# lxmeng/mms_answer_selection

Hardware: AMD Instinct MI355X
Metric: QA pairs/sec (fwd+bwd) at batch 4096, 300-d; % HBM roofline (higher is better)
Workload: dtype f32

## Files before the change

mms_answer_selection_amd/csrc/euclid_math.h:

```cpp
#ifndef MMS_EUCLID_MATH_H_
#define MMS_EUCLID_MATH_H_

#include <hip/hip_runtime.h>

#include "mms_common.h"

namespace mms {

struct EuclidCoef {
  float c;
  double den;
  double rcp;
};

__device__ __forceinline__ double rcp_newton(double den) {
  double r = __builtin_amdgcn_rcp(den);
  r = __builtin_fma(__builtin_fma(-den, r, 1.0), r, r);
  r = __builtin_fma(__builtin_fma(-den, r, 1.0), r, r);
  return r;
}

__device__ __forceinline__ EuclidCoef euclid_coef(float T, float g) {
  EuclidCoef k;
  k.c = g * T * T * T;
// ... 132 lines not shown
inline void with_glove_d4(int D, F&& f) {
  switch (D) {
    case 100: f(std::integral_constant<int, 25>{}); break;
    case 200: f(std::integral_constant<int, 50>{}); break;
    case 300: f(std::integral_constant<int, 75>{}); break;
  }
}
inline bool wave_width_ok(int D) { return D <= 1024; }
inline int wave_pairs(int D) { return D <= 400 ? 2 : 1; }

template <int LPR> struct SpecPlan;
template <> struct SpecPlan<32> { static constexpr int H1 = 12, L1 = 13, H2 = 15; };
template <> struct SpecPlan<64> { static constexpr int H1 = 25, L1 = 26, H2 = 36; };

template <int LPR>
__device__ __forceinline__ float chain_sum_speculative(const float4* img4, int D4, float pred1,
                                                       float pred2, int j, int lead) {
  typedef SpecPlan<LPR> P;
  const int h4 = spec_h4(D4);
  const int seg = (j == 0) ? 0 : (j <= P::L1 ? 1 : 2);
  const int c0 = (seg == 1) ? 2 * (j - 1) - P::H1 : 2 * (j - 1 - P::L1) - P::H2;
  const int pbits = __float_as_int(seg == 1 ? pred1 : pred2);
  float2v start;
  start.x = (seg == 0) ? 0.0f : __int_as_float(pbits + c0);
  start.y = (seg == 0) ? 0.0f : __int_as_float(pbits + c0 + 1);
  __builtin_amdgcn_s_setprio(3);
  const float2v end = chain_sum_lds_pk(img4 + seg * h4, h4, start);
  const float s1 = __shfl(end.x, lead, 64);
  const int k1 = __float_as_int(s1) - __float_as_int(pred1) + P::H1;
  const bool hit1 = (k1 >= 0) && (k1 <= 2 * P::H1);
  const int l1 = lead + 1 + ((hit1 ? k1 : 0) >> 1);
  const float e1x = __shfl(end.x, l1, 64), e1y = __shfl(end.y, l1, 64);
  float s2 = (k1 & 1) ? e1y : e1x;
  if (!hit1) s2 = chain_sum_lds(img4 + h4, h4, s1);
  const int k2 = __float_as_int(s2) - __float_as_int(pred2) + P::H2;
  const bool hit2 = (k2 >= 0) && (k2 <= 2 * P::H2);
  const int l2 = lead + 1 + P::L1 + ((hit2 ? k2 : 0) >> 1);
  const float e2x = __shfl(end.x, l2, 64), e2y = __shfl(end.y, l2, 64);
  float s3 = (k2 & 1) ? e2y : e2x;
  if (!hit2) s3 = chain_sum_lds(img4 + 2 * h4, h4, s2);
  __builtin_amdgcn_s_setprio(0);
  return s3;
}

typedef __attribute__((address_space(3))) const mms_v4f lds_v4f;
__device__ __forceinline__ unsigned lds_address(const void* p) {
  return (unsigned)(size_t)(__attribute__((address_space(3))) const void*)p;
}
__device__ __forceinline__ float4 lds_read4(unsigned addr, int u) {
  const mms_v4f t = ((lds_v4f*)(size_t)addr)[u];
  return make_float4(t.x, t.y, t.z, t.w);
}

template <int H4>
struct SpecSegment {
  float4 v[H4];
  __device__ __forceinline__ void load(const float4* r4) {
#pragma unroll
    for (int u = 0; u < H4; ++u) v[u] = r4[u];
  }
  __device__ __forceinline__ float2v chain(float2v s) const {
#pragma unroll
    for (int u = 0; u < H4; ++u) {
      const float2v lo = {v[u].x, v[u].y}, hi = {v[u].z, v[u].w};
      s = s + __builtin_shufflevector(lo, lo, 0, 0);
      s = s + __builtin_shufflevector(lo, lo, 1, 1);
      s = s + __builtin_shufflevector(hi, hi, 0, 0);
      s = s + __builtin_shufflevector(hi, hi, 1, 1);
    }
    return s;
  }

  static constexpr int AHEAD = H4 < 15 ? H4 : 15;
  __device__ __forceinline__ void load_first(unsigned seg) {
#pragma unroll
    for (int u = 0; u < AHEAD; ++u) v[u] = lds_read4(seg, u);
  }
  __device__ __forceinline__ float2v chain_streamed(unsigned seg, float2v s) {
#pragma unroll
    for (int u = 0; u < H4; ++u) {
      const float2v lo = {v[u].x, v[u].y}, hi = {v[u].z, v[u].w};
      s = __builtin_shufflevector(lo, lo, 0, 0) + s;
      s = __builtin_shufflevector(lo, lo, 1, 1) + s;
      s = __builtin_shufflevector(hi, hi, 0, 0) + s;
      s = __builtin_shufflevector(hi, hi, 1, 1) + s;
      if (u + AHEAD < H4) {
        asm volatile("" : "+v"(seg) : "v"(s));
        v[u + AHEAD] = lds_read4(seg, u + AHEAD);
      }
      __builtin_amdgcn_sched_barrier(0);
    }
    return s;
  }
};

__device__ __forceinline__ int spec_seg32(int j) { return (j == 0) ? 0 : (j <= SpecPlan<32>::L1 ? 1 : 2); }

__device__ __forceinline__ float2v spec_start32(float pred1, float pred2, int j) {
  typedef SpecPlan<32> P;
  const int seg = spec_seg32(j);
  const int c0 = (seg == 1) ? 2 * (j - 1) - P::H1 : 2 * (j - 1 - P::L1) - P::H2;
  const int pbits = __float_as_int(seg == 1 ? pred1 : pred2);
  float2v start;
  start.x = (seg == 0) ? 0.0f : __int_as_float(pbits + c0);
  start.y = (seg == 0) ? 0.0f : __int_as_float(pbits + c0 + 1);
  return start;
// ... 26 lines not shown
```

mms_answer_selection_amd/csrc/simcross_rows.hip:

```cpp
#include <atomic>
#include <cstdlib>
#include <cstring>

#include "cosine_math.h"
#include "euclid_math.h"
#include "mms_internal.h"

namespace mms {

template <int NIT, int RW, bool FWD, bool BWD>
__global__ __launch_bounds__(256) void euclid_rows_wave_kernel(
    const float* __restrict__ q, const float* __restrict__ a,
    const float* __restrict__ top_in, const float* __restrict__ top_diff,
    float* __restrict__ top_out, float* __restrict__ dq, float* __restrict__ da, int N,
    int D4) {
  constexpr int LPR = 64 / RW;
  extern __shared__ float4 lds4[];
  const int wave = threadIdx.x >> 6, lane = threadIdx.x & 63;
  const int row0 = (blockIdx.x * 4 + wave) * RW;
  if (row0 >= N) return;
  const int rows = min(RW, N - row0);
  const int n4 = rows * D4;
  const size_t base4 = (size_t)row0 * D4;
  const float4* q4 = reinterpret_cast<const float4*>(q) + base4;
// ... 53 lines not shown
    wave_lds_sync();
    const float dist = chain_sum_speculative<LPR>(sq4 + grow * st4, D4, my1, my2, j, grp * LPR);
    T = 1.0f / (1.0f + sqrtf(dist));
    if (BWD) asm volatile("" : "+v"(g));
    if (j == 0 && grp < rows) top_out[row0 + grp] = T;
  }
  if (!BWD) return;

  const EuclidCoef mine = euclid_coef(T, g);
  EuclidCoef kr[RW];
#pragma unroll
  for (int r = 0; r < RW; ++r) {
    kr[r].c = __int_as_float(__builtin_amdgcn_readlane(__float_as_int(mine.c), r * LPR));
    {
      const long long dn = __double_as_longlong(mine.den), rc = __double_as_longlong(mine.rcp);
      const unsigned dlo = __builtin_amdgcn_readlane((int)(unsigned)dn, r * LPR);
      const unsigned dhi = __builtin_amdgcn_readlane((int)(unsigned)(dn >> 32), r * LPR);
      const unsigned rlo = __builtin_amdgcn_readlane((int)(unsigned)rc, r * LPR);
      const unsigned rhi = __builtin_amdgcn_readlane((int)(unsigned)(rc >> 32), r * LPR);
      kr[r].den = __longlong_as_double((long long)(((unsigned long long)dhi << 32) | dlo));
      kr[r].rcp = __longlong_as_double((long long)(((unsigned long long)rhi << 32) | rlo));
    }
  }
  float4* dq4 = reinterpret_cast<float4*>(dq) + base4;
  float4* da4 = reinterpret_cast<float4*>(da) + base4;
  float4 t[NIT];
  bool any_risky = false;
#pragma unroll
  for (int it = 0; it < NIT; ++it) {
    const int i = lane + 64 * it;
    const EuclidCoef& k = (RW == 2 && i >= D4) ? kr[RW - 1] : kr[0];
    bool risky;
    t[it] = euclid_tt4_fast(k, df[it], risky);
    any_risky |= risky && (i < n4);
  }
  if (any_risky) {
#pragma unroll
    for (int it = 0; it < NIT; ++it) {
      const int i = lane + 64 * it;
      const EuclidCoef& k = (RW == 2 && i >= D4) ? kr[RW - 1] : kr[0];
      t[it] = euclid_tt4_exact(k, df[it]);
    }
  }
#pragma unroll
  for (int it = 0; it < NIT; ++it) {
    const int i = lane + 64 * it;
    if (i >= n4) break;
    float4 o0, o1;
    o0.x = 0.f + t[it].x; o0.y = 0.f + t[it].y; o0.z = 0.f + t[it].z; o0.w = 0.f + t[it].w;
    o1.x = 0.f + (-t[it].x); o1.y = 0.f + (-t[it].y); o1.z = 0.f + (-t[it].z); o1.w = 0.f + (-t[it].w);
    stream_store(dq4 + i, o0);
    stream_store(da4 + i, o1);
  }
}

template <typename I>
__device__ __forceinline__ float4 load4(const float4* p, I i) {
  const mms_v4f v = reinterpret_cast<const mms_v4f*>(p)[i];
  return make_float4(v.x, v.y, v.z, v.w);
}

template <int D4C, int WPB, bool SHIFT, bool FULL>
__device__ __forceinline__ void euclid_pair32_forward(int N, const float* __restrict__ q, const float* __restrict__ a,
                                                      float* __restrict__ top_out, float4* lds4) {
  constexpr int NIT = (D4C + 31) / 32;
  constexpr int H4 = (D4C + 2) / 3, ST4 = 3 * H4;
  constexpr int MAXU = SHIFT ? 7 : 0;
  constexpr int P1_LAST = (H4 + MAXU - 1) / 32 < NIT - 1 ? (H4 + MAXU - 1) / 32 : NIT - 1;
  constexpr int P2_LAST = (2 * H4 + MAXU - 1) / 32 < NIT - 1 ? (2 * H4 + MAXU - 1) / 32 : NIT - 1;
  const int wave = threadIdx.x >> 6, lane = threadIdx.x & 63;
  const int grp = lane >> 5, j = lane & 31;
  const int want = (blockIdx.x * WPB + wave) * 2 + grp;
  const bool have = FULL || want < N;
  const int row = have ? want : N - 1;
  const unsigned r0 = (unsigned)row * D4C;
  const float4* q4 = reinterpret_cast<const float4*>(q) + (FULL ? 0 : (size_t)row * D4C);
  const float4* a4 = reinterpret_cast<const float4*>(a) + (FULL ? 0 : (size_t)row * D4C);
  const int u = !SHIFT ? 0
                : FULL ? (int)(((unsigned)(reinterpret_cast<size_t>(q) >> 4) + r0) & 7)
                       : (int)((reinterpret_cast<size_t>(q4) >> 4) & 7);
  const int j0 = j - u;
  const bool first_ok = !SHIFT || j0 >= 0;
  const bool last_ok = j0 + 32 * (NIT - 1) < D4C;
  auto valid_slot = [&](int it) { return (it > 0 || first_ok) && (it < NIT - 1 || last_ok); };

  float4 x[NIT], y[NIT];
#pragma unroll
  for (int it = 0; it < NIT; ++it) {
    const int i = valid_slot(it) ? j0 + 32 * it : 0;
    if constexpr (FULL) {
      const unsigned off = (r0 + (unsigned)i) * 16u;
      const char* qb = reinterpret_cast<const char*>(q4) + off;
      const char* ab = reinterpret_cast<const char*>(a4) + off;
      x[it] = load4(reinterpret_cast<const float4*>(qb), 0);
      y[it] = load4(reinterpret_cast<const float4*>(ab), 0);
    } else {
      x[it] = load4(q4, i);
      y[it] = load4(a4, i);
    }
    __builtin_amdgcn_sched_barrier(0);
  }

  float4* img = lds4 + (wave * 2 + grp) * ST4;
  unsigned seg = lds_address(img + spec_seg32(j) * H4);
  asm volatile("" : "+v"(seg));
  if (ST4 > D4C && j < ST4 - D4C) img[D4C + j] = make_float4(0.f, 0.f, 0.f, 0.f);
  float p1 = 0.f, p2 = 0.f;
  float2v start = {0.f, 0.f};
#pragma unroll
  for (int it = 0; it < NIT; ++it) {
    const bool valid = valid_slot(it);
    float4 s;
// ... 998 lines not shown
```

mms_answer_selection_amd/csrc/triplet_steps.hip:

```cpp
#include <cmath>
#include <cstdint>

#include "cosine_math.h"
#include "euclid_math.h"
#include "pairrank_math.h"
#include "mms_internal.h"

namespace mms {

constexpr int kTicketTop = 1024;
constexpr int kTicketStride = kTicketTop + 32;
constexpr int kTicketGroup = 16;
constexpr int kFxSumBits = 52;
constexpr int kFxTermBits = 10;
constexpr unsigned long long kFxPoison = 1ull << 63;
constexpr unsigned long long kFxOne = 1ull << kFxSumBits;
constexpr unsigned long long kFxSumMask = kFxOne - 1;

static thread_local int t_triplet_finish = MMS_TRIPLET_FINISH_INLAUNCH;
int triplet_finish_mode() { return t_triplet_finish; }
void set_triplet_finish_mode(int m) { t_triplet_finish = m; }

struct LossArrival {
  unsigned long long fx_sum = 0, fx_bad = 0;
  bool top_wait = false;
  unsigned long long top_old = 0, top_pay = 0;
  __device__ __forceinline__ void add(float tm, double fx_scale) {
    const bool ok = tm >= 0.f && tm < (float)(1 << kFxTermBits);
    fx_sum += ok ? (unsigned long long)((double)tm * fx_scale) : 0ull;
    fx_bad += ok ? 0ull : 1ull;
  }
  template <int WPB>
  __device__ __forceinline__ void arrive(unsigned long long* wg_arrivals, unsigned long long* __restrict__ ticket) {
    const unsigned long long pay = (1ull << 60) | (fx_bad ? kFxOne : 0ull) | fx_sum;
    const unsigned long long old = __hip_atomic_fetch_add(wg_arrivals, pay, __ATOMIC_RELAXED, __HIP_MEMORY_SCOPE_WORKGROUP);
    if ((old >> 60) == (unsigned long long)(WPB - 1)) {
      const unsigned long long wg = old + pay;
      const unsigned grp = blockIdx.x / kTicketGroup;
      const unsigned gsize = min((unsigned)kTicketGroup, gridDim.x - (unsigned)kTicketGroup * grp);
      const unsigned long long gpay = kFxOne | (wg & kFxSumMask);
      if ((wg >> kFxSumBits) & 0xffull)
        __hip_atomic_fetch_or(ticket + grp, kFxPoison, __ATOMIC_RELAXED, __HIP_MEMORY_SCOPE_AGENT);
      const unsigned long long gold = __hip_atomic_fetch_add(ticket + grp, gpay, __ATOMIC_RELAXED, __HIP_MEMORY_SCOPE_AGENT);
      if (((gold >> kFxSumBits) & 0x7ffull) == (unsigned long long)(gsize - 1)) {
        const unsigned long long g = gold + gpay;
        __hip_atomic_store(ticket + grp, 0ull, __ATOMIC_RELAXED, __HIP_MEMORY_SCOPE_AGENT);
        top_pay = kFxOne | (g & kFxSumMask);
        if (g & kFxPoison) __hip_atomic_fetch_or(ticket + kTicketTop, kFxPoison, __ATOMIC_RELAXED, __HIP_MEMORY_SCOPE_AGENT);
        top_old = __hip_atomic_fetch_add(ticket + kTicketTop, top_pay, __ATOMIC_RELAXED, __HIP_MEMORY_SCOPE_AGENT);
        top_wait = true;
      }
    }
  }
  __device__ __forceinline__ void finish(unsigned long long* __restrict__ ticket, float* __restrict__ loss, double fx_scale,
// ... 56 lines not shown
    predp1 += (i < h4) ? a4 : 0.f; predp2 += (i < 2 * h4) ? a4 : 0.f;
    predn1 += (i < h4) ? b4 : 0.f; predn2 += (i < 2 * h4) ? b4 : 0.f;
  }
  {
    const int npad = st4 - D4;
    if (lane < 2 * npad) sqp[(lane / npad) * st4 + D4 + (lane % npad)] = make_float4(0.f, 0.f, 0.f, 0.f);
  }
  const int br = lane >> 5, j = lane & 31;
  float dist;
  if (SPEC) {
    predp1 = wave_sum(predp1); predp2 = wave_sum(predp2);
    predn1 = wave_sum(predn1); predn2 = wave_sum(predn2);
    wave_lds_sync();
    dist = chain_sum_speculative<32>(br ? sqn : sqp, D4, br ? predn1 : predp1, br ? predn2 : predp2,
                                     j, br * 32);
  } else {
    wave_lds_sync();
    dist = 0.f;
    if (j == 0) {
      dist = chain_sum_lds(br ? sqn : sqp, st4, 0.f);
    }
    dist = __shfl(dist, br * 32, 64);
  }
  const float Tmine = 1.0f / (1.0f + sqrtf(dist));
  const float Tp = __shfl(Tmine, 0, 64), Tn = __shfl(Tmine, 32, 64);
  asm volatile("" : "+v"(yy));
  if (lane == 0) { s_pos[row] = Tp; s_neg[row] = Tn; }

  const PairTerm pt = pair_term(Tp, Tn, yy, margin);
  float ga, gb;
  pair_grad(yy, pt.ordered, pt.similar, s0, s1, ga, gb, hinge_ge != 0);
  if (lane == 0) partials[row] = pt.term;
  const EuclidCoef k0 = euclid_coef(Tp, ga), k1 = euclid_coef(Tn, gb);

  float4* dq4 = reinterpret_cast<float4*>(dq) + base4;
  float4* dp4 = reinterpret_cast<float4*>(dap) + base4;
  float4* dn4 = reinterpret_cast<float4*>(dan) + base4;
#pragma unroll
  for (int it = 0; it < NIT; ++it) {
    const int i = lane + 64 * it;
    if (i >= D4) break;
    const float4 tp = euclid_tt4(k0, dp[it]), tn = euclid_tt4(k1, dn[it]);
    float4 oq, op, on;
    oq.x = (0.f + tp.x) + (0.f + tn.x); oq.y = (0.f + tp.y) + (0.f + tn.y);
    oq.z = (0.f + tp.z) + (0.f + tn.z); oq.w = (0.f + tp.w) + (0.f + tn.w);
    op.x = 0.f + (-tp.x); op.y = 0.f + (-tp.y); op.z = 0.f + (-tp.z); op.w = 0.f + (-tp.w);
    on.x = 0.f + (-tn.x); on.y = 0.f + (-tn.y); on.z = 0.f + (-tn.z); on.w = 0.f + (-tn.w);
    stream_store(dq4 + i, oq);
    stream_store(dp4 + i, op);
    stream_store(dn4 + i, on);
  }
}

template <int D4C, bool EXACT, int WPB, bool INL>
__global__ __launch_bounds__(64 * WPB) void triplet32x2_kernel(
    int N, float margin, float s0, float s1, const float* __restrict__ q,
    const float* __restrict__ ap, const float* __restrict__ an, const float* __restrict__ y,
    float* __restrict__ s_pos, float* __restrict__ s_neg, float* __restrict__ partials,
    float* __restrict__ dq, float* __restrict__ dap, float* __restrict__ dan, int hinge_ge,
    unsigned long long* __restrict__ ticket, float* __restrict__ loss, double fx_scale) {
  constexpr int C = 2 * D4C;
  constexpr int NIT = (C + 63) / 64;
  constexpr int PNIT = (D4C + 31) / 32, LASTN = D4C - 32 * (PNIT - 1);
  constexpr int H4 = (D4C + 2) / 3, ST4 = 3 * H4;
  __shared__ float4 lds4[WPB * 4 * ST4];
  __shared__ unsigned long long wg_arrivals;
  const int wave = threadIdx.x >> 6, lane = threadIdx.x & 63;
  if (INL) {
    if (threadIdx.x == 0) wg_arrivals = 0;
    asm volatile("s_waitcnt lgkmcnt(0)\n\ts_barrier" ::: "memory");
  }
  const long long r0 = ((long long)blockIdx.x * WPB + wave) * 2;
  const long long total4 = (long long)N * D4C;
  const long long b4 = r0 * D4C;
  const float4* q4 = reinterpret_cast<const float4*>(q);
  const float4* p4 = reinterpret_cast<const float4*>(ap);
  const float4* m4 = reinterpret_cast<const float4*>(an);
  float yy[2];
#pragma unroll
  for (int t = 0; t < 2; ++t) yy[t] = y[min(r0 + t, (long long)N - 1)];
  float4 dp[NIT], dn[NIT];
  {
    float4 x[NIT], u[NIT], v[NIT];
#pragma unroll
    for (int it = 0; it < NIT; ++it) {
      const int i = lane + 64 * it;
      long long gi = b4 + ((NIT * 64 == C || i < C) ? i : 0);
      gi = gi < total4 ? gi : total4 - 1;
      x[it] = q4[gi]; u[it] = p4[gi]; v[it] = m4[gi];
    }
    float4* img = lds4 + (size_t)wave * 4 * ST4;
#pragma unroll
    for (int it = 0; it < NIT; ++it) {
      const int i = lane + 64 * it;
      dp[it].x = x[it].x - u[it].x; dp[it].y = x[it].y - u[it].y;
      dp[it].z = x[it].z - u[it].z; dp[it].w = x[it].w - u[it].w;
      dn[it].x = x[it].x - v[it].x; dn[it].y = x[it].y - v[it].y;
      dn[it].z = x[it].z - v[it].z; dn[it].w = x[it].w - v[it].w;
      float4 a, b;
      a.x = dp[it].x * dp[it].x; a.y = dp[it].y * dp[it].y;
      a.z = dp[it].z * dp[it].z; a.w = dp[it].w * dp[it].w;
      b.x = dn[it].x * dn[it].x; b.y = dn[it].y * dn[it].y;
      b.z = dn[it].z * dn[it].z; b.w = dn[it].w * dn[it].w;
      if (NIT * 64 == C || i < C) {
        const int t = i >= D4C ? 1 : 0, c = i - t * D4C;
        img[(2 * t) * ST4 + c] = a;
        img[(2 * t + 1) * ST4 + c] = b;
      }
    }
    if constexpr (ST4 > D4C) {
      if (lane < 4 * (ST4 - D4C))
        img[(lane / (ST4 - D4C)) * ST4 + D4C + lane % (ST4 - D4C)] = make_float4(0.f, 0.f, 0.f, 0.f);
    }
  }
  asm volatile("" : "+v"(yy[0]), "+v"(yy[1]));
  wave_lds_sync();

  const int br = lane >> 5, j = lane & 31;
  float4* dq4 = reinterpret_cast<float4*>(dq);
  float4* dp4 = reinterpret_cast<float4*>(dap);
  float4* dn4 = reinterpret_cast<float4*>(dan);
  constexpr bool LATE = INL;
  LossArrival arr;
  EuclidCoef k0[2], k1[2];
  float c0[2] = {0.f, 0.f}, c1[2] = {0.f, 0.f}, rr0[2] = {0.f, 0.f}, rr1[2] = {0.f, 0.f};
  auto store_pass = [&](int t) {
    const bool have = r0 + t < N;
#pragma unroll
    for (int it = 0; it < NIT; ++it) {
      if (64 * it >= (t + 1) * D4C || 64 * it + 63 < t * D4C) continue;
      const int i = lane + 64 * it;
      const bool mine = have && i >= t * D4C && i < (t + 1) * D4C;
      float4 tp, tn;
      if (EXACT) { tp = euclid_tt4(k0[t], dp[it]); tn = euclid_tt4(k1[t], dn[it]); }
      else {
        tp.x = (c0[t] * dp[it].x) * rr0[t]; tp.y = (c0[t] * dp[it].y) * rr0[t];
        tp.z = (c0[t] * dp[it].z) * rr0[t]; tp.w = (c0[t] * dp[it].w) * rr0[t];
        tn.x = (c1[t] * dn[it].x) * rr1[t]; tn.y = (c1[t] * dn[it].y) * rr1[t];
        tn.z = (c1[t] * dn[it].z) * rr1[t]; tn.w = (c1[t] * dn[it].w) * rr1[t];
      }
      if (mine) {
        float4 oq, op, on;
        oq.x = (0.f + tp.x) + (0.f + tn.x); oq.y = (0.f + tp.y) + (0.f + tn.y);
        oq.z = (0.f + tp.z) + (0.f + tn.z); oq.w = (0.f + tp.w) + (0.f + tn.w);
        op.x = 0.f + (-tp.x); op.y = 0.f + (-tp.y); op.z = 0.f + (-tp.z); op.w = 0.f + (-tp.w);
        on.x = 0.f + (-tn.x); on.y = 0.f + (-tn.y); on.z = 0.f + (-tn.z); on.w = 0.f + (-tn.w);
        stream_store(dq4 + b4 + i, oq);
        stream_store(dp4 + b4 + i, op);
        stream_store(dn4 + b4 + i, on);
      }
    }
  };
#pragma unroll
  for (int t = 0; t < 2; ++t) {
    const bool have = r0 + t < N;
    const long long row = have ? r0 + t : (long long)N - 1;
    const float4* im = lds4 + ((size_t)wave * 4 + 2 * t + br) * ST4;
    SpecSegment<H4> sg;
    sg.load(im + spec_seg32(j) * H4);
    const bool last_ok = (LASTN >= 32) || (j < LASTN);
    float p1 = 0.f, p2 = 0.f;
#pragma unroll
    for (int it = 0; it < PNIT; ++it) {
      const bool valid = (it < PNIT - 1) || last_ok;
      const float4 sq = im[valid ? j + 32 * it : 0];
      const float s4 = valid ? (sq.x + sq.y) + (sq.z + sq.w) : 0.f;
      const int i = j + 32 * it;
      if (32 * it + 31 < H4) p1 += s4;
      else if (32 * it < H4) p1 += (i < H4) ? s4 : 0.f;
      if (32 * it + 31 < 2 * H4) p2 += s4;
      else if (32 * it < 2 * H4) p2 += (i < 2 * H4) ? s4 : 0.f;
    }
    p1 = half_wave_sum(p1);
    p2 = half_wave_sum(p2);
    __builtin_amdgcn_s_setprio(3);
    const float2v start = spec_start32(p1, p2, j);
    const float2v end = sg.chain(start);
    bool hit;
    float dist = spec_resolve_halves(start, end, j, &hit);
    if (!hit) {
      dist = chain_sum_lds(im, ST4, 0.0f);
    }
    __builtin_amdgcn_s_setprio(0);
    const float Tmine = 1.0f / (1.0f + sqrtf(dist));
    const float Tp = __int_as_float(__builtin_amdgcn_readlane(__float_as_int(Tmine), 0));
    const float Tn = __int_as_float(__builtin_amdgcn_readlane(__float_as_int(Tmine), 32));
    const PairTerm pt = pair_term(Tp, Tn, yy[t], margin);
    float ga, gb;
    pair_grad(yy[t], pt.ordered, pt.similar, s0, s1, ga, gb, hinge_ge != 0);
    if (EXACT) { k0[t] = euclid_coef(Tp, ga); k1[t] = euclid_coef(Tn, gb); }
    else {
      c0[t] = ga * Tp * Tp * Tp; c1[t] = gb * Tn * Tn * Tn;
      rr0[t] = (float)rcp_newton((double)(Tp - 1.0f) + 1e-9);
      rr1[t] = (float)rcp_newton((double)(Tn - 1.0f) + 1e-9);
    }
    if (INL) {
      arr.add(have ? pt.term : 0.f, fx_scale);
      if (t == 1 && lane == 0) arr.template arrive<WPB>(&wg_arrivals, ticket);
    } else {
      if (lane == 0 && have) partials[row] = pt.term;
    }
    if (lane == 0 && have) { s_pos[row] = Tp; s_neg[row] = Tn; }
    if (!LATE) store_pass(t);
  }
  if (LATE) { store_pass(0); store_pass(1); }
  if (!INL) return;
  arr.finish(ticket, loss, fx_scale, N);
}

template <int ROWS, int THREADS>
__global__ __launch_bounds__(THREADS) void triplet_generic_kernel(
    int N, int D, float margin, float s0, float s1, const float* __restrict__ q,
    const float* __restrict__ ap, const float* __restrict__ an, const float* __restrict__ y,
    float* __restrict__ s_pos, float* __restrict__ s_neg, float* __restrict__ partials,
    float* __restrict__ dq, float* __restrict__ dap, float* __restrict__ dan, int hinge_ge) {
  extern __shared__ float4 lds_raw[];
  float* dpos = reinterpret_cast<float*>(lds_raw);
  float* dneg = dpos + (size_t)ROWS * D;
  __shared__ float Ts[2][ROWS];
  __shared__ float cs[2][ROWS];
  __shared__ double dens[2][ROWS];
  __shared__ float terms[ROWS];

  const int row0 = blockIdx.x * ROWS;
  const int rows = min(ROWS, N - row0);
  if (rows <= 0) return;
  const size_t base = (size_t)row0 * D;
  const int total = rows * D;
  for (int i = threadIdx.x; i < total; i += THREADS) {
    const float x = q[base + i];
    dpos[i] = x - ap[base + i];
    dneg[i] = x - an[base + i];
  }
  __syncthreads();
  if (threadIdx.x < 2 * ROWS) {
    const int br = threadIdx.x / ROWS, r = threadIdx.x % ROWS;
    if (r < rows) {
      const float* src = (br ? dneg : dpos) + r * D;
      float dist = 0.f;
      for (int d = 0; d < D; ++d) dist += src[d] * src[d];
      const float T = 1.0f / (1.0f + sqrtf(dist));
      Ts[br][r] = T;
      (br ? s_neg : s_pos)[row0 + r] = T;
    }
  }
  __syncthreads();
  if (threadIdx.x < ROWS) {
    const int r = threadIdx.x;
    float t = 0.f;
    if (r < rows) {
      const float yy = y[row0 + r];
      const PairTerm p = pair_term(Ts[0][r], Ts[1][r], yy, margin);
      float ga, gb;
      pair_grad(yy, p.ordered, p.similar, s0, s1, ga, gb, hinge_ge != 0);
      const EuclidCoef k0 = euclid_coef(Ts[0][r], ga), k1 = euclid_coef(Ts[1][r], gb);
      cs[0][r] = k0.c; dens[0][r] = k0.den;
      cs[1][r] = k1.c; dens[1][r] = k1.den;
      t = p.term;
    }
    terms[r] = t;
// ... 10 lines not shown
  }
}

constexpr int kTripRows = 8;
constexpr int kTripThreads = 256;

constexpr size_t kTicketBytes = (size_t)kTicketStride * sizeof(unsigned long long);

size_t triplet_workspace_bytes(int N) { return kTicketBytes + (size_t)N * sizeof(float); }

int triplet_workspace_init(void* ws, size_t ws_bytes, hipStream_t s) {
  if (ws == nullptr || ws_bytes < kTicketBytes || (reinterpret_cast<uintptr_t>(ws) & 7u)) return MMS_ERR_WORKSPACE;
  return hipMemsetAsync(ws, 0, kTicketBytes, s) == hipSuccess ? MMS_OK : MMS_ERR_LAUNCH;
}

struct TripletPlan {
  float s0, s1;
  int hge;
  unsigned long long* tickets;
  float* partials;
};
static int triplet_plan(int N, float loss_weight, void* ws, size_t ws_bytes, TripletPlan* p) {
  if (ws == nullptr || ws_bytes < triplet_workspace_bytes(N) || (reinterpret_cast<uintptr_t>(ws) & 7u))
    return MMS_ERR_WORKSPACE;
  const float scale = loss_weight / (float)N;
  *p = {-1.0f * scale, 1.0f * scale, pairrank_hinge_mode() == MMS_PAIRRANK_HINGE_GPU ? 1 : 0,
        static_cast<unsigned long long*>(ws), reinterpret_cast<float*>(static_cast<char*>(ws) + kTicketBytes)};
  return MMS_OK;
}

struct InLaunchLoss { unsigned long long* tickets; double fx_scale; };
static InLaunchLoss in_launch_loss(const TripletPlan& p, unsigned grid, int N, const float* loss) {
  const unsigned ngrp = (grid + kTicketGroup - 1) / kTicketGroup;
  const bool inl = triplet_finish_mode() == MMS_TRIPLET_FINISH_INLAUNCH && ngrp <= (unsigned)kTicketTop &&
                   loss_sum_mode() != MMS_LOSS_SUM_REFERENCE && loss != nullptr;
  int lg = 0;
  while (((long long)1 << lg) < (long long)N) ++lg;
  return {inl ? p.tickets : nullptr, std::ldexp(1.0, kFxSumBits - kFxTermBits - lg)};
}

int triplet_euclid_step(int N, int D, float margin, float loss_weight, const float* q,
                        const float* ap, const float* an, const float* y, float* s_pos,
                        float* s_neg, float* loss, float* dq, float* dap, float* dan, void* ws,
                        size_t ws_bytes, hipStream_t s) {
  if (N == 0) return MMS_OK;
  TripletPlan p;
  if (const int rc = triplet_plan(N, loss_weight, ws, ws_bytes, &p)) return rc;
  const bool v = (D % 4 == 0) && aligned16(q) && aligned16(ap) && aligned16(an) &&
                 aligned16(dq) && aligned16(dap) && aligned16(dan);
  if (v && glove_width(D)) {
    constexpr int WPB = 8;
    const unsigned grid = (unsigned)((N + WPB * 2 - 1) / (WPB * 2));
    const InLaunchLoss il = in_launch_loss(p, grid, N, loss);
    with_glove_d4(D, [&](auto W) {
      with_bool(euclid_backward_mode() == MMS_EUCLID_BWD_REFERENCE, [&](auto EXACT) {
        with_bool(il.tickets != nullptr, [&](auto INL) {
          hipLaunchKernelGGL((triplet32x2_kernel<decltype(W)::value, decltype(EXACT)::value, WPB, decltype(INL)::value>),
                             dim3(grid), dim3(64 * WPB), 0, s, N, margin, p.s0, p.s1, q, ap, an, y, s_pos, s_neg,
                             p.partials, dq, dap, dan, p.hge, il.tickets, loss, il.fx_scale);
        });
      });
    });
    if (il.tickets) return launch_status();
  } else if (v && wave_width_ok(D)) {
    const int D4 = D / 4;
    const int nit = (D4 + 63) / 64;
    const unsigned grid = (unsigned)((N + 3) / 4);
    const size_t lds = spec_image_lds(4, 2, D4);
    const bool spec = wave_pairs(D) == 2;
    static constexpr decltype(&triplet_wave_kernel<1, true>) kernels[2][4] = {MMS_NIT4(triplet_wave_kernel, false),
                                                                              MMS_NIT4(triplet_wave_kernel, true)};
    hipLaunchKernelGGL(kernels[spec][nit - 1], dim3(grid), dim3(256), lds, s, N, D4, margin, p.s0, p.s1, q, ap, an, y,
                       s_pos, s_neg, p.partials, dq, dap, dan, p.hge);
  } else {
    const size_t lds = 2 * (size_t)kTripRows * D * sizeof(float);
    if (lds > 96 * 1024) return MMS_ERR_UNSUPPORTED;
    hipLaunchKernelGGL((triplet_generic_kernel<kTripRows, kTripThreads>), dim3((unsigned)((N + kTripRows - 1) / kTripRows)),
                       dim3(kTripThreads), lds, s, N, D, margin, p.s0, p.s1, q, ap, an, y, s_pos,
                       s_neg, p.partials, dq, dap, dan, p.hge);
  }
  if (loss == nullptr) return launch_status();
  return triplet_loss_from_terms(p.partials, N, loss, s);
}

template <int D4C, int WPB, bool INL, bool VOUT>
__global__ __launch_bounds__(64 * WPB) void triplet_cosine32_kernel(
    int N, float margin, float s0, float s1, const float* __restrict__ q,
    const float* __restrict__ ap, const float* __restrict__ an, const float* __restrict__ y,
    float* __restrict__ s_pos, float* __restrict__ s_neg, float* __restrict__ norm_q,
    float* __restrict__ norm_pos, float* __restrict__ norm_neg, float* __restrict__ partials,
    float* __restrict__ dq, float* __restrict__ dap, float* __restrict__ dan, int hinge_ge,
    unsigned long long* __restrict__ ticket, float* __restrict__ loss, double fx_scale) {
  constexpr int NIT = (D4C + 31) / 32;
  __shared__ unsigned long long wg_arrivals;
  const int wave = threadIdx.x >> 6, lane = threadIdx.x & 63, grp = lane >> 5, j = lane & 31;
  if (INL) {
    if (threadIdx.x == 0) wg_arrivals = 0;
    asm volatile("s_waitcnt lgkmcnt(0)\n\ts_barrier" ::: "memory");
  }
  const long long want = ((long long)blockIdx.x * WPB + wave) * 2 + grp;
  const bool have = want < N;
  const long long row = have ? want : (long long)N - 1;
  const float4* q4 = reinterpret_cast<const float4*>(q) + row * D4C;
  const float4* p4 = reinterpret_cast<const float4*>(ap) + row * D4C;
  const float4* m4 = reinterpret_cast<const float4*>(an) + row * D4C;
  float4 x[NIT], u[NIT], v[NIT];
#pragma unroll
  for (int it = 0; it < NIT; ++it) {
    const int i = j + 32 * it;
    const int ii = i < D4C ? i : 0;
    x[it] = q4[ii]; u[it] = p4[ii]; v[it] = m4[ii];
  }
// ... 225 lines not shown
```

Measured before the change: 591.1 million.

## Restructure triplet euclid kernel to overlap prefix sums, LDS chain and stores

The triplet32x2 kernel is reorganised so that all global loads are issued up front, before the LDS barrier. The per-pair partial sums are now computed in registers while the squares are being written to LDS, instead of re-reading LDS afterwards. The first pair's stores are interleaved with the second pair's chain, and a FULL specialisation with 32-bit address arithmetic drops bounds clamps when N divides evenly. The aim is to hide load and LDS latency and cut address and compare work, at the cost of more register pressure and more template instantiations.

```diff
diff --git a/mms_answer_selection_amd/csrc/euclid_math.h b/mms_answer_selection_amd/csrc/euclid_math.h
--- a/mms_answer_selection_amd/csrc/euclid_math.h
+++ b/mms_answer_selection_amd/csrc/euclid_math.h
@@ -208,6 +208,12 @@
   return make_float4(t.x, t.y, t.z, t.w);
 }
 
+template <typename I>
+__device__ __forceinline__ float4 load4(const float4* p, I i) {
+  const mms_v4f v = reinterpret_cast<const mms_v4f*>(p)[i];
+  return make_float4(v.x, v.y, v.z, v.w);
+}
+
 template <int H4>
 struct SpecSegment {
   float4 v[H4];
diff --git a/mms_answer_selection_amd/csrc/simcross_rows.hip b/mms_answer_selection_amd/csrc/simcross_rows.hip
--- a/mms_answer_selection_amd/csrc/simcross_rows.hip
+++ b/mms_answer_selection_amd/csrc/simcross_rows.hip
@@ -129,12 +129,6 @@
     stream_store(dq4 + i, o0);
     stream_store(da4 + i, o1);
   }
-}
-
-template <typename I>
-__device__ __forceinline__ float4 load4(const float4* p, I i) {
-  const mms_v4f v = reinterpret_cast<const mms_v4f*>(p)[i];
-  return make_float4(v.x, v.y, v.z, v.w);
 }
 
 template <int D4C, int WPB, bool SHIFT, bool FULL>
diff --git a/mms_answer_selection_amd/csrc/triplet_steps.hip b/mms_answer_selection_amd/csrc/triplet_steps.hip
--- a/mms_answer_selection_amd/csrc/triplet_steps.hip
+++ b/mms_answer_selection_amd/csrc/triplet_steps.hip
@@ -1,5 +1,6 @@
 #include <cmath>
 #include <cstdint>
+#include <type_traits>
 
 #include "cosine_math.h"
 #include "euclid_math.h"
@@ -162,7 +163,15 @@
   }
 }
 
-template <int D4C, bool EXACT, int WPB, bool INL>
+template <int A, int B, class F>
+__device__ __forceinline__ void static_for(F&& f) {
+  if constexpr (A < B) {
+    f(std::integral_constant<int, A>{});
+    static_for<A + 1, B>(f);
+  }
+}
+
+template <int D4C, bool EXACT, int WPB, bool INL, bool FULL = false>
 __global__ __launch_bounds__(64 * WPB) void triplet32x2_kernel(
     int N, float margin, float s0, float s1, const float* __restrict__ q,
     const float* __restrict__ ap, const float* __restrict__ an, const float* __restrict__ y,
@@ -170,152 +179,226 @@
     float* __restrict__ dq, float* __restrict__ dap, float* __restrict__ dan, int hinge_ge,
     unsigned long long* __restrict__ ticket, float* __restrict__ loss, double fx_scale) {
   constexpr int C = 2 * D4C;
-  constexpr int NIT = (C + 63) / 64;
-  constexpr int PNIT = (D4C + 31) / 32, LASTN = D4C - 32 * (PNIT - 1);
+  constexpr int NIT = (C + 63) / 64, LAST = NIT - 1;
   constexpr int H4 = (D4C + 2) / 3, ST4 = 3 * H4;
+  constexpr int CL0 = (2 * H4 - 1) / 64, CL1 = (D4C + 2 * H4 - 1) / 64;
+  constexpr int PS0 = (D4C - 1) / 64, PS1 = LAST;
   __shared__ float4 lds4[WPB * 4 * ST4];
   __shared__ unsigned long long wg_arrivals;
   const int wave = threadIdx.x >> 6, lane = threadIdx.x & 63;
+  const int br = lane >> 5, j = lane & 31;
+  const long long r0 = ((long long)blockIdx.x * WPB + wave) * 2;
+  const long long total4 = (long long)N * D4C;
+  const long long b4 = r0 * D4C;
+  const bool have[2] = {FULL || r0 < N, FULL || r0 + 1 < N};
+  auto in_run = [](int it, int i) { return NIT * 64 == C || it < LAST || i < C; };
+  auto at = [&](auto* base, int i) {
+    using T = std::remove_pointer_t<decltype(base)>;
+    if constexpr (FULL) {
+      using B = std::conditional_t<std::is_const_v<T>, const char, char>;
+      return reinterpret_cast<T*>(reinterpret_cast<B*>(base) + ((unsigned)b4 + (unsigned)i) * 16u);
+    } else {
+      return base + (b4 + i);
+    }
+  };
+
+  float yy[2];
+#pragma unroll
+  for (int t = 0; t < 2; ++t) yy[t] = FULL ? y[(unsigned)r0 + t] : y[min(r0 + t, (long long)N - 1)];
+  const float4* q4 = reinterpret_cast<const float4*>(q);
+  const float4* p4 = reinterpret_cast<const float4*>(ap);
+  const float4* m4 = reinterpret_cast<const float4*>(an);
+  float4 x[NIT], u[NIT], v[NIT];
+#pragma unroll
+  for (int it = 0; it < NIT; ++it) {
+    const int i = lane + 64 * it;
+    const int ci = in_run(it, i) ? i : 0;
+    if constexpr (FULL) {
+      x[it] = load4(at(q4, ci), 0); u[it] = load4(at(p4, ci), 0); v[it] = load4(at(m4, ci), 0);
+    } else {
+      long long gi = b4 + ci;
+      gi = gi < total4 ? gi : total4 - 1;
+      x[it] = load4(q4, gi); u[it] = load4(p4, gi); v[it] = load4(m4, gi);
+    }
+    __builtin_amdgcn_sched_barrier(0);
+  }
+  asm volatile("" :: "s"(s_pos), "s"(s_neg), "s"(partials), "s"(dq), "s"(dap), "s"(dan), "s"(hinge_ge), "s"(ticket),
+               "s"(loss), "s"(fx_scale));
   if (INL) {
     if (threadIdx.x == 0) wg_arrivals = 0;
     asm volatile("s_waitcnt lgkmcnt(0)\n\ts_barrier" ::: "memory");
-  }
-  const long long r0 = ((long long)blockIdx.x * WPB + wave) * 2;
-  const long long total4 = (long long)N * D4C;
-  const long long b4 = r0 * D4C;
-  const float4* q4 = reinterpret_cast<const float4*>(q);
-  const float4* p4 = reinterpret_cast<const float4*>(ap);
-  const float4* m4 = reinterpret_cast<const float4*>(an);
-  float yy[2];
-#pragma unroll
-  for (int t = 0; t < 2; ++t) yy[t] = y[min(r0 + t, (long long)N - 1)];
+    __builtin_amdgcn_sched_barrier(0);
+  }
+  float4* img = lds4 + (size_t)wave * 4 * ST4;
+  unsigned seg[2];
+#pragma unroll
+  for (int t = 0; t < 2; ++t) {
+    seg[t] = lds_address(img + (2 * t + br) * ST4 + spec_seg32(j) * H4);
+    asm volatile("" : "+v"(seg[t]));
+  }
+  if constexpr (ST4 > D4C) {
+    if (lane < 4 * (ST4 - D4C))
+      img[(lane / (ST4 - D4C)) * ST4 + D4C + lane % (ST4 - D4C)] = make_float4(0.f, 0.f, 0.f, 0.f);
+  }
+
   float4 dp[NIT], dn[NIT];
-  {
-    float4 x[NIT], u[NIT], v[NIT];
-#pragma unroll
-    for (int it = 0; it < NIT; ++it) {
-      const int i = lane + 64 * it;
-      long long gi = b4 + ((NIT * 64 == C || i < C) ? i : 0);
-      gi = gi < total4 ? gi : total4 - 1;
-      x[it] = q4[gi]; u[it] = p4[gi]; v[it] = m4[gi];
-    }
-    float4* img = lds4 + (size_t)wave * 4 * ST4;
-#pragma unroll
-    for (int it = 0; it < NIT; ++it) {
-      const int i = lane + 64 * it;
-      dp[it].x = x[it].x - u[it].x; dp[it].y = x[it].y - u[it].y;
-      dp[it].z = x[it].z - u[it].z; dp[it].w = x[it].w - u[it].w;
-      dn[it].x = x[it].x - v[it].x; dn[it].y = x[it].y - v[it].y;
-      dn[it].z = x[it].z - v[it].z; dn[it].w = x[it].w - v[it].w;
-      float4 a, b;
-      a.x = dp[it].x * dp[it].x; a.y = dp[it].y * dp[it].y;
-      a.z = dp[it].z * dp[it].z; a.w = dp[it].w * dp[it].w;
-      b.x = dn[it].x * dn[it].x; b.y = dn[it].y * dn[it].y;
-      b.z = dn[it].z * dn[it].z; b.w = dn[it].w * dn[it].w;
-      if (NIT * 64 == C || i < C) {
-        const int t = i >= D4C ? 1 : 0, c = i - t * D4C;
-        img[(2 * t) * ST4 + c] = a;
-        img[(2 * t + 1) * ST4 + c] = b;
+  float ca1[2] = {0.f, 0.f}, ca2[2] = {0.f, 0.f}, cb1[2] = {0.f, 0.f}, cb2[2] = {0.f, 0.f};
+  float2v start[2] = {{0.f, 0.f}, {0.f, 0.f}};
+  auto centre = [&](int t) {
+    const float p1 = half_wave_sum(swap_halves_add(ca1[t], cb1[t]));
+    const float p2 = half_wave_sum(swap_halves_add(ca2[t], cb2[t]));
+    start[t] = spec_start32(p1, p2, j);
+    asm volatile("" : "+v"(start[t]));
+  };
+  auto slot = [&](auto IT) __attribute__((always_inline)) {
+    constexpr int it = decltype(IT)::value;
+    const int i = lane + 64 * it;
+    dp[it].x = x[it].x - u[it].x; dp[it].y = x[it].y - u[it].y;
+    dp[it].z = x[it].z - u[it].z; dp[it].w = x[it].w - u[it].w;
+    dn[it].x = x[it].x - v[it].x; dn[it].y = x[it].y - v[it].y;
+    dn[it].z = x[it].z - v[it].z; dn[it].w = x[it].w - v[it].w;
+    float4 a, b;
+    a.x = dp[it].x * dp[it].x; a.y = dp[it].y * dp[it].y;
+    a.z = dp[it].z * dp[it].z; a.w = dp[it].w * dp[it].w;
+    b.x = dn[it].x * dn[it].x; b.y = dn[it].y * dn[it].y;
+    b.z = dn[it].z * dn[it].z; b.w = dn[it].w * dn[it].w;
+    asm volatile("" : "+v"(a.x), "+v"(a.y), "+v"(a.z), "+v"(a.w), "+v"(b.x), "+v"(b.y), "+v"(b.z), "+v"(b.w));
+    if (in_run(it, i)) {
+      const int t = i >= D4C ? 1 : 0, c = i - t * D4C;
+      img[(2 * t) * ST4 + c] = a;
+      img[(2 * t + 1) * ST4 + c] = b;
+    }
+    const float a4 = (a.x + a.y) + (a.z + a.w), b4s = (b.x + b.y) + (b.z + b.w);
+#pragma unroll
+    for (int t = 0; t < 2; ++t) {
+      const int lo = t * D4C, c = i - lo;
+      if (64 * it + 63 >= lo && 64 * it < lo + H4) {
+        const bool in1 = c >= 0 && c < H4;
+        ca1[t] += in1 ? a4 : 0.f; cb1[t] += in1 ? b4s : 0.f;
       }
-    }
-    if constexpr (ST4 > D4C) {
-      if (lane < 4 * (ST4 - D4C))
-        img[(lane / (ST4 - D4C)) * ST4 + D4C + lane % (ST4 - D4C)] = make_float4(0.f, 0.f, 0.f, 0.f);
-    }
-  }
-  asm volatile("" : "+v"(yy[0]), "+v"(yy[1]));
-  wave_lds_sync();
-
-  const int br = lane >> 5, j = lane & 31;
+      if (64 * it + 63 >= lo && 64 * it < lo + 2 * H4) {
+        const bool in2 = c >= 0 && c < 2 * H4;
+        ca2[t] += in2 ? a4 : 0.f; cb2[t] += in2 ? b4s : 0.f;
+      }
+    }
+    if (it == CL0 && CL0 < PS0) centre(0);
+    if (it == CL1 && CL1 > PS0 && CL1 < PS1) centre(1);
+    __builtin_amdgcn_sched_barrier(0);
+  };
+
+  LossArrival arr;
+  float Tp[2], Tn[2], term[2];
+  EuclidCoef k0[2], k1[2];
+  float c0[2] = {0.f, 0.f}, c1[2] = {0.f, 0.f}, rr0[2] = {0.f, 0.f}, rr1[2] = {0.f, 0.f};
+  auto pass_begin = [&](auto TT, SpecSegment<H4>& sg) __attribute__((always_inline)) {
+    constexpr int t = decltype(TT)::value;
+    wave_lds_sync();
+    __builtin_amdgcn_s_setprio(3);
+    sg.load_first(seg[t]);
+    if (t == 0 && CL0 >= PS0) centre(0);
+    if ((t == 0 && CL1 <= PS0) || (t == 1 && CL1 >= PS1)) centre(1);
+  };
+  auto pass_end = [&](auto TT, SpecSegment<H4>& sg) __attribute__((always_inline)) {
+    constexpr int t = decltype(TT)::value;
+    const float2v end = sg.chain_streamed(seg[t], start[t]);
+    bool hit;
+    float dist = spec_resolve_halves(start[t], end, j, &hit);
+    if (!hit) {
+      dist = chain_sum_lds(img + (2 * t + br) * ST4, ST4, 0.0f);
+    }
+    __builtin_amdgcn_s_setprio(0);
+    const float Tmine = 1.0f / (1.0f + sqrtf(dist));
+    Tp[t] = __int_as_float(__builtin_amdgcn_readlane(__float_as_int(Tmine), 0));
+    Tn[t] = __int_as_float(__builtin_amdgcn_readlane(__float_as_int(Tmine), 32));
+    const PairTerm pt = pair_term(Tp[t], Tn[t], yy[t], margin);
+    float ga, gb;
+    pair_grad(yy[t], pt.ordered, pt.similar, s0, s1, ga, gb, hinge_ge != 0);
+    term[t] = pt.term;
+    if constexpr (EXACT) {
+      k0[t] = euclid_coef(Tp[t], ga); k1[t] = euclid_coef(Tn[t], gb);
+      asm volatile("" : "+v"(k0[t].c), "+v"(k0[t].den), "+v"(k0[t].rcp), "+v"(k1[t].c), "+v"(k1[t].den), "+v"(k1[t].rcp));
+    } else {
+      c0[t] = ga * Tp[t] * Tp[t] * Tp[t]; c1[t] = gb * Tn[t] * Tn[t] * Tn[t];
+      rr0[t] = (float)rcp_newton((double)(Tp[t] - 1.0f) + 1e-9);
+      rr1[t] = (float)rcp_newton((double)(Tn[t] - 1.0f) + 1e-9);
+      asm volatile("" : "+v"(c0[t]), "+v"(c1[t]), "+v"(rr0[t]), "+v"(rr1[t]));
+    }
+    if (INL) arr.add(have[t] ? pt.term : 0.f, fx_scale);
+    __builtin_amdgcn_sched_barrier(0);
+  };
+
   float4* dq4 = reinterpret_cast<float4*>(dq);
   float4* dp4 = reinterpret_cast<float4*>(dap);
   float4* dn4 = reinterpret_cast<float4*>(dan);
+  auto stored_in = [](int it) { return 64 * it + 63 >= D4C ? 1 : 0; };
+  auto store_slot = [&](auto IT) __attribute__((always_inline)) {
+    constexpr int it = decltype(IT)::value;
+    constexpr bool both = 64 * it < D4C && 64 * it + 63 >= D4C;
+    constexpr int ts = 64 * it >= D4C ? 1 : 0;
+    const int i = lane + 64 * it;
+    const bool second = both && i >= D4C;
+    float4 tp, tn;
+    if constexpr (EXACT) {
+      EuclidCoef ka = k0[ts], kb = k1[ts];
+      if constexpr (both) {
+        ka.c = second ? k0[1].c : k0[0].c; ka.den = second ? k0[1].den : k0[0].den; ka.rcp = second ? k0[1].rcp : k0[0].rcp;
+        kb.c = second ? k1[1].c : k1[0].c; kb.den = second ? k1[1].den : k1[0].den; kb.rcp = second ? k1[1].rcp : k1[0].rcp;
+      }
+      tp = euclid_tt4(ka, dp[it]); tn = euclid_tt4(kb, dn[it]);
+    } else {
+      float ca = c0[ts], ra = rr0[ts], cb = c1[ts], rb = rr1[ts];
+      if constexpr (both) {
+        ca = second ? c0[1] : c0[0]; ra = second ? rr0[1] : rr0[0];
+        cb = second ? c1[1] : c1[0]; rb = second ? rr1[1] : rr1[0];
+      }
+      tp.x = (ca * dp[it].x) * ra; tp.y = (ca * dp[it].y) * ra;
+      tp.z = (ca * dp[it].z) * ra; tp.w = (ca * dp[it].w) * ra;
+      tn.x = (cb * dn[it].x) * rb; tn.y = (cb * dn[it].y) * rb;
+      tn.z = (cb * dn[it].z) * rb; tn.w = (cb * dn[it].w) * rb;
+    }
+    const bool live = in_run(it, i) && (FULL || b4 + i < total4);
+    if (live) {
+      float4 oq, op, on;
+      oq.x = (0.f + tp.x) + (0.f + tn.x); oq.y = (0.f + tp.y) + (0.f + tn.y);
+      oq.z = (0.f + tp.z) + (0.f + tn.z); oq.w = (0.f + tp.w) + (0.f + tn.w);
+      op.x = 0.f + (-tp.x); op.y = 0.f + (-tp.y); op.z = 0.f + (-tp.z); op.w = 0.f + (-tp.w);
+      on.x = 0.f + (-tn.x); on.y = 0.f + (-tn.y); on.z = 0.f + (-tn.z); on.w = 0.f + (-tn.w);
+      stream_store(at(dq4, i), oq);
+      stream_store(at(dp4, i), op);
+      stream_store(at(dn4, i), on);
+    }
+    if constexpr (FULL) __builtin_amdgcn_sched_barrier(0);
+  };
+  auto store_pass = [&](auto TT) __attribute__((always_inline)) {
+    constexpr int t = decltype(TT)::value;
+    if (lane == 0 && have[t]) {
+      s_pos[r0 + t] = Tp[t]; s_neg[r0 + t] = Tn[t];
+      if (!INL) partials[r0 + t] = term[t];
+    }
+    static_for<0, NIT>([&](auto IT) {
+      if constexpr (stored_in(decltype(IT)::value) == t) store_slot(IT);
+    });
+  };
+
   constexpr bool LATE = INL;
-  LossArrival arr;
-  EuclidCoef k0[2], k1[2];
-  float c0[2] = {0.f, 0.f}, c1[2] = {0.f, 0.f}, rr0[2] = {0.f, 0.f}, rr1[2] = {0.f, 0.f};
-  auto store_pass = [&](int t) {
-    const bool have = r0 + t < N;
-#pragma unroll
-    for (int it = 0; it < NIT; ++it) {
-      if (64 * it >= (t + 1) * D4C || 64 * it + 63 < t * D4C) continue;
-      const int i = lane + 64 * it;
-      const bool mine = have && i >= t * D4C && i < (t + 1) * D4C;
-      float4 tp, tn;
-      if (EXACT) { tp = euclid_tt4(k0[t], dp[it]); tn = euclid_tt4(k1[t], dn[it]); }
-      else {
-        tp.x = (c0[t] * dp[it].x) * rr0[t]; tp.y = (c0[t] * dp[it].y) * rr0[t];
-        tp.z = (c0[t] * dp[it].z) * rr0[t]; tp.w = (c0[t] * dp[it].w) * rr0[t];
-        tn.x = (c1[t] * dn[it].x) * rr1[t]; tn.y = (c1[t] * dn[it].y) * rr1[t];
-        tn.z = (c1[t] * dn[it].z) * rr1[t]; tn.w = (c1[t] * dn[it].w) * rr1[t];
-      }
-      if (mine) {
-        float4 oq, op, on;
-        oq.x = (0.f + tp.x) + (0.f + tn.x); oq.y = (0.f + tp.y) + (0.f + tn.y);
-        oq.z = (0.f + tp.z) + (0.f + tn.z); oq.w = (0.f + tp.w) + (0.f + tn.w);
-        op.x = 0.f + (-tp.x); op.y = 0.f + (-tp.y); op.z = 0.f + (-tp.z); op.w = 0.f + (-tp.w);
-        on.x = 0.f + (-tn.x); on.y = 0.f + (-tn.y); on.z = 0.f + (-tn.z); on.w = 0.f + (-tn.w);
-        stream_store(dq4 + b4 + i, oq);
-        stream_store(dp4 + b4 + i, op);
-        stream_store(dn4 + b4 + i, on);
-      }
-    }
-  };
-#pragma unroll
-  for (int t = 0; t < 2; ++t) {
-    const bool have = r0 + t < N;
-    const long long row = have ? r0 + t : (long long)N - 1;
-    const float4* im = lds4 + ((size_t)wave * 4 + 2 * t + br) * ST4;
+  asm volatile("" : "+v"(yy[0]), "+v"(yy[1]));
+  static_for<0, PS0 + 1>(slot);
+  {
     SpecSegment<H4> sg;
-    sg.load(im + spec_seg32(j) * H4);
-    const bool last_ok = (LASTN >= 32) || (j < LASTN);
-    float p1 = 0.f, p2 = 0.f;
-#pragma unroll
-    for (int it = 0; it < PNIT; ++it) {
-      const bool valid = (it < PNIT - 1) || last_ok;
-      const float4 sq = im[valid ? j + 32 * it : 0];
-      const float s4 = valid ? (sq.x + sq.y) + (sq.z + sq.w) : 0.f;
-      const int i = j + 32 * it;
-      if (32 * it + 31 < H4) p1 += s4;
-      else if (32 * it < H4) p1 += (i < H4) ? s4 : 0.f;
-      if (32 * it + 31 < 2 * H4) p2 += s4;
-      else if (32 * it < 2 * H4) p2 += (i < 2 * H4) ? s4 : 0.f;
-    }
-    p1 = half_wave_sum(p1);
-    p2 = half_wave_sum(p2);
-    __builtin_amdgcn_s_setprio(3);
-    const float2v start = spec_start32(p1, p2, j);
-    const float2v end = sg.chain(start);
-    bool hit;
-    float dist = spec_resolve_halves(start, end, j, &hit);
-    if (!hit) {
-      dist = chain_sum_lds(im, ST4, 0.0f);
-    }
-    __builtin_amdgcn_s_setprio(0);
-    const float Tmine = 1.0f / (1.0f + sqrtf(dist));
-    const float Tp = __int_as_float(__builtin_amdgcn_readlane(__float_as_int(Tmine), 0));
-    const float Tn = __int_as_float(__builtin_amdgcn_readlane(__float_as_int(Tmine), 32));
-    const PairTerm pt = pair_term(Tp, Tn, yy[t], margin);
-    float ga, gb;
-    pair_grad(yy[t], pt.ordered, pt.similar, s0, s1, ga, gb, hinge_ge != 0);
-    if (EXACT) { k0[t] = euclid_coef(Tp, ga); k1[t] = euclid_coef(Tn, gb); }
-    else {
-      c0[t] = ga * Tp * Tp * Tp; c1[t] = gb * Tn * Tn * Tn;
-      rr0[t] = (float)rcp_newton((double)(Tp - 1.0f) + 1e-9);
-      rr1[t] = (float)rcp_newton((double)(Tn - 1.0f) + 1e-9);
-    }
-    if (INL) {
-      arr.add(have ? pt.term : 0.f, fx_scale);
-      if (t == 1 && lane == 0) arr.template arrive<WPB>(&wg_arrivals, ticket);
-    } else {
-      if (lane == 0 && have) partials[row] = pt.term;
-    }
-    if (lane == 0 && have) { s_pos[row] = Tp; s_neg[row] = Tn; }
-    if (!LATE) store_pass(t);
-  }
-  if (LATE) { store_pass(0); store_pass(1); }
-  if (!INL) return;
-  arr.finish(ticket, loss, fx_scale, N);
+    pass_begin(std::integral_constant<int, 0>{}, sg);
+    pass_end(std::integral_constant<int, 0>{}, sg);
+  }
+  static_for<PS0 + 1, NIT>(slot);
+  {
+    SpecSegment<H4> sg;
+    pass_begin(std::integral_constant<int, 1>{}, sg);
+    if constexpr (!LATE) store_pass(std::integral_constant<int, 0>{});
+    pass_end(std::integral_constant<int, 1>{}, sg);
+  }
+  if (INL && lane == 0) arr.template arrive<WPB>(&wg_arrivals, ticket);
+  if constexpr (LATE) store_pass(std::integral_constant<int, 0>{});
+  store_pass(std::integral_constant<int, 1>{});
+  if (INL) arr.finish(ticket, loss, fx_scale, N);
 }
 
 template <int ROWS, int THREADS>
@@ -432,12 +515,16 @@
     constexpr int WPB = 8;
     const unsigned grid = (unsigned)((N + WPB * 2 - 1) / (WPB * 2));
     const InLaunchLoss il = in_launch_loss(p, grid, N, loss);
+    const bool full = N % (2 * WPB) == 0 && (unsigned long long)N * D * sizeof(float) <= 0xffffffffull;
     with_glove_d4(D, [&](auto W) {
       with_bool(euclid_backward_mode() == MMS_EUCLID_BWD_REFERENCE, [&](auto EXACT) {
         with_bool(il.tickets != nullptr, [&](auto INL) {
-          hipLaunchKernelGGL((triplet32x2_kernel<decltype(W)::value, decltype(EXACT)::value, WPB, decltype(INL)::value>),
-                             dim3(grid), dim3(64 * WPB), 0, s, N, margin, p.s0, p.s1, q, ap, an, y, s_pos, s_neg,
-                             p.partials, dq, dap, dan, p.hge, il.tickets, loss, il.fx_scale);
+          with_bool(full, [&](auto FULL) {
+            hipLaunchKernelGGL((triplet32x2_kernel<decltype(W)::value, decltype(EXACT)::value, WPB, decltype(INL)::value,
+                                                   decltype(FULL)::value>),
+                               dim3(grid), dim3(64 * WPB), 0, s, N, margin, p.s0, p.s1, q, ap, an, y, s_pos, s_neg,
+                               p.partials, dq, dap, dan, p.hge, il.tickets, loss, il.fx_scale);
+          });
         });
       });
     });
```

Result: no change. 594.0 million, median of 5 (+0.5%).
